# sundy-li/databend

Hardware: AMD Instinct MI355X
Metric: input rows/sec aggregated (filter + hash GROUP BY), % HBM roofline (higher is better)
Workload: dtype int16 key / u64 count; 1 GPU; clickbench_q8_adv_engine_id; rows_per_gpu=100000000, input_copies=4, groups=32, selected_rows=629660, parallelism=single

## Files before the change

databend_amd/csrc/abi.hip:

```cpp
#include "abi_internal.hpp"

static thread_local std::string g_last_error;

int fail(int code, const std::string& msg) {
    g_last_error = msg;
    return code;
}
int abi_fail(int code, const std::string& msg) { return fail(code, msg); }

int err_bits_fail(u64 err, u64 mask) {
    err &= mask;
    if (err & ERR_OVF_LOST) return fail(DBG_ERR_INTERNAL, "overflow list exhausted");
    if (err & ERR_MINMAX_SPIN)
        return fail(DBG_ERR_INTERNAL, "Decimal128 MIN/MAX: a state update gave up after 2^20 contended attempts (the result would be wrong)");
    if (err & ERR_CHAIN_SPIN)
        return fail(DBG_ERR_INTERNAL, "fused finalize: a parked row was not posted in time (GPU hand-off stalled)");
    if (err & ERR_FIXED_INCOMPLETE)
        return fail(DBG_ERR_INVALID, "fixed-capacity exchange incomplete (a partial held more groups than the "
                                     "buffer, or unresolved overflow): use dbg_agg_partition + export_records");
    return DBG_OK;
}

int own_alloc(Owner o, size_t bytes) {
    DevBuf b;
// ... 431 lines not shown
        hipError_t e = hipGetDevice(&h->device);
        if (e != hipSuccess) {
            delete h;
            return fail(DBG_ERR_DEVICE, std::string("hipGetDevice: ") + hipGetErrorString(e));
        }
    }
    auto cleanup = [&](int code) {
        dbg_agg_destroy(h);
        return code;
    };
    if (hipSetDevice(h->device) != hipSuccess) return cleanup(fail(DBG_ERR_DEVICE, "hipSetDevice failed"));
    if (hipStreamCreateWithFlags(&h->own_stream, hipStreamNonBlocking) != hipSuccess) return cleanup(fail(DBG_ERR_DEVICE, "hipStreamCreate failed"));
    h->stream = h->own_stream;
    if ((rc = h->counters.ensure(CNT_WORDS)) != DBG_OK) return cleanup(rc);
    if (hipMemset(h->counters, 0, CNT_WORDS * 8) != hipSuccess) return cleanup(fail(DBG_ERR_DEVICE, "memset"));
    h->spec.err = h->counters + CNT_ERR;
    {
        const char* cx = getenv("DBG_X_PPSPEC_CAP");
        const char* fd = getenv("DBG_X_PPSPEC_DESC");
        h->spec.x_pp_cap = cx ? std::max<u32>(64, (u32)atoi(cx) & ~3u) : ~0u;
        h->spec.x_pp_desc = (fd && fd[0] == '1') ? 1 : 0;
    }
    if ((rc = h->dspec.ensure(1)) != DBG_OK) return cleanup(rc);
    if (hipMemcpy(h->dspec, &h->spec, sizeof(Spec), hipMemcpyHostToDevice) != hipSuccess) return cleanup(fail(DBG_ERR_DEVICE, "spec upload"));
    if ((rc = h->hcounters.ensure(CNT_WORDS + DBG_MAX_KEYS + 8)) != DBG_OK) return cleanup(rc);
    if (hipHostGetDevicePointer((void**)&h->hcounters_dev, h->hcounters.get(), 0) != hipSuccess) h->hcounters_dev = nullptr;
    h->hint_groups = params->capacity_hint;
    u64 hint = params->capacity_hint ? params->capacity_hint : 512;
    h->cap = pow2_at_least(std::max<u64>(hint * 2, 1024));
    h->init_cap = h->cap;
    if ((rc = alloc_table(h, h->cap, h->slots)) != DBG_OK) return cleanup(rc);
    h->scr_blocks = DBG_INSERT_MAX_BLOCKS;
    if ((rc = h->scratch.ensure(scr_words(h->scr_blocks, (u32)h->spec.stride_words))) != DBG_OK) return cleanup(rc);
    if (hipMemset(h->scratch, 0, (size_t)h->scr_blocks * 16) != hipSuccess) return cleanup(fail(DBG_ERR_DEVICE, "memset"));

    BatchDesc* st;
    u32 bid;
    if ((rc = new_batch(h, &st, &bid)) != DBG_OK) return cleanup(rc);
    h->n_batches = 0;
    if (hipStreamSynchronize(h->stream) != hipSuccess) return cleanup(fail(DBG_ERR_DEVICE, "sync"));
    *out = h;
    return DBG_OK;
}

void dbg_agg_destroy(dbg_agg_handle* h) {
    if (!h) return;
    hipSetDevice(h->device);
    if (h->stream) hipStreamSynchronize(h->stream);
    if (h->switch_ev) hipEventDestroy(h->switch_ev);
    if (h->own_stream) hipStreamDestroy(h->own_stream);
    delete h;
}

int dbg_agg_set_stream(dbg_agg_handle* h, void* s) {
    if (!h) return fail(DBG_ERR_INVALID, "null handle");
    HIPCHECK(hipSetDevice(h->device));
    RETURN_IF(flush_deferred(h));
    hipStream_t ns = s ? (hipStream_t)s : h->own_stream;
    if (ns != h->stream) {
        if (!h->switch_ev) HIPCHECK(hipEventCreateWithFlags(&h->switch_ev, hipEventDisableTiming));
        HIPCHECK(hipEventRecord(h->switch_ev, h->stream));
        HIPCHECK(hipStreamWaitEvent(ns, h->switch_ev, 0));
        h->stream = ns;
    }
    return DBG_OK;
}

// ... 132 lines not shown
```

databend_amd/csrc/abi_finalize.hip:

```cpp
#include "abi_exp.hpp"

static void note_observed(dbg_agg_handle* h) {
    const u64 rows = h->table_rows > h->remerged ? h->table_rows - h->remerged : 0;
    if (h->pp || !rows) return;
    h->obs_rows = rows;
    h->obs_groups = h->n_groups;
}

static void publish_groups(const dbg_agg_handle* h, uint64_t* n_groups, uint64_t* string_bytes) {
    if (n_groups) *n_groups = h->n_groups;
    if (string_bytes)
        for (int c = 0; c < h->spec.n_keys; ++c) string_bytes[c] = h->string_bytes[c];
}

bool groups_known(dbg_agg_handle* h, u64 groups, const u64* str_tot, const FinState* caps, uint64_t* n_groups,
                  uint64_t* string_bytes) {
    const Spec& S = h->spec;
    h->n_groups = groups;
    note_observed(h);
    h->string_bytes.assign(S.n_keys, 0);
    bool short_buf = caps && groups > caps->max_groups;
    for (int c = 0; c < S.n_keys; ++c) {
        if (S.key_types[c].type != DBG_STRING) continue;
        h->string_bytes[c] = str_tot[c];
// ... 150 lines not shown
        const u64 total = (size_t)a < h->agg_string_bytes.size() ? h->agg_string_bytes[a] : 0;
        if (on_device && (!out_aggs[a].offsets || (total && !out_aggs[a].data)))
            return fail(DBG_ERR_INVALID, "dbg_agg_result: a String aggregate needs offsets and data buffers");
        u64* offs = nullptr;
        u8* data = nullptr;
        if (dest(out_aggs[a].offsets, (n + 1) * 8, (void**)&offs) != DBG_OK || dest(out_aggs[a].data, total, (void**)&data) != DBG_OK)
            return DBG_ERR_OOM;
        {
            prof::Scope ps("str_gather", h->stream);
            launch_str_gather(h->stream, h->dbatches, a, (const u64*)od.agg_data[a], n, offs, data, total);
        }
        to_host(out_aggs[a].offsets, offs, (n + 1) * 8);
        to_host(out_aggs[a].data, data, total);
    }
    for (int a = 0; a < S.n_aggs && !ser; ++a)
        if (h->result_types[a].nullable) RETURN_IF(pack_validity(od.agg_valid[a], out_aggs[a]));
    for (int c = 0; c < S.n_keys; ++c) {
        const dbg_datatype& t = S.key_types[c];
        to_host(out_keys[c].data, od.key_data[c], t.type == DBG_STRING ? h->string_bytes[c] : n * type_width(t.type));
        if (t.type == DBG_STRING) to_host(out_keys[c].offsets, od.key_offsets[c], (n + 1) * 8);
    }
    for (int a = 0; a < S.n_aggs && !ser; ++a)
        if (!is_str_minmax(S.aggs[a])) to_host(out_aggs[a].data, od.agg_data[a], n * type_width(h->result_types[a].type));
    HIPCHECK(hipMemcpyAsync(h->hcounters, h->counters, CNT_WORDS * 8, hipMemcpyDeviceToHost, h->stream));
    hipError_t e = hipStreamSynchronize(h->stream);
    if (e != hipSuccess) return fail(DBG_ERR_DEVICE, std::string("result: ") + hipGetErrorString(e));
    if (h->hcounters[CNT_ERR] & ERR_DEC_OVERFLOW) {
        HIPCHECK(hipMemsetAsync(h->counters + CNT_ERR, 0, 8, h->stream));
        return fail(DBG_ERR_OVERFLOW, "Decimal overflow");
    }
    return DBG_OK;
}

static int fin_launch(dbg_agg_handle* h) {
    FinState& F = h->fin;
    const Spec& S = h->spec;
    RETURN_IF(stage_flush(h));
    u64 nb = finalize_blocks(h->cap);
    RETURN_IF(h->d_pos.ensure(nb + 16, 1024));
    RETURN_IF(h->d_str_pos.ensure((u64)S.n_keys * nb + 8, 1024));
    const bool direct = h->def_part && !h->pp && S.n_keys == 1 && S.n_aggs == 1 && !S.key_types[0].nullable &&
                        !h->result_types[0].nullable && type_width(h->result_types[0].type) == 8 && F.keys[0].data && F.aggs[0].data &&
                        type_width(S.key_types[0].type) == (u32)h->def_part_kw;
    if (direct) {
        h->def_part = false;
        RETURN_IF(h->part_status.ensure(part_direct_status_words(h->cap, h->def_part_sb), 1024));
    }
    TableDesc t = direct ? TableDesc{} : table_desc(h);
    const bool small = h->cap + 1 <= FIN_SMALL_SLOTS;
    const bool fuse = h->def_on && !h->pp && small && h->hcounters_dev && insert_can_fuse(S, h->def_hb, h->cap);
    if (!fuse) RETURN_IF(flush_deferred(h));
    u64* totals = h->d_pos + nb;
    F.direct = direct;
    if (!small && !h->pp && !direct) count_and_scan(h, t, nb);
    OutDesc od;
    memset(&od, 0, sizeof(od));
    od.cap_groups = F.max_groups;
    u8* vb = h->vbytes;
    for (int c = 0; c < S.n_keys; ++c) {
        od.key_data[c] = F.keys[c].data;
        od.key_offsets[c] = S.key_types[c].type == DBG_STRING ? F.keys[c].offsets : nullptr;
        od.cap_str[c] = (S.key_types[c].type == DBG_STRING && F.has_max_str) ? F.max_str[c] : 0;
        F.cap_str[c] = od.cap_str[c];
        if (S.key_types[c].nullable) {
            od.key_valid[c] = vb;
            od.key_bits[c] = F.keys[c].validity;
            vb += F.max_groups + 1;
        }
    }
    for (int a = 0; a < S.n_aggs; ++a) {
        od.agg_data[a] = F.aggs[a].data;
        if (h->result_types[a].nullable) {
            od.agg_bits[a] = F.aggs[a].validity;
            if (agg_always_valid(S.aggs[a])) {
                od.all_valid |= 1u << a;
            } else {
                od.agg_valid[a] = vb;
                vb += F.max_groups + 1;
            }
        }
    }
    if (h->pp) {
        F.zero_copy = false;
        F.seq = ++h->fin_seq;
        RETURN_IF(pp_fin_launch(h, od));
        F.active = true;
        return DBG_OK;
    }
    F.zero_copy = small && !direct && h->hcounters_dev != nullptr;
    F.seq = ++h->fin_seq;
    if (direct) {
        prof::Scope ps("part_direct", h->stream);
        TableDesc td{};
        td.slots = h->slots;
        td.cap = h->cap;
        hipError_t e = launch_part_direct(h->stream, td, h->def_part_sb, h->part_sorted, h->part_bounds, h->part_status,
                                          h->def_part_kw, od.key_data[0], (u64*)od.agg_data[0], od.cap_groups, totals);
        if (e != hipSuccess) return fail(DBG_ERR_DEVICE, std::string("partitioned insert (direct stage): ") + hipGetErrorString(e));
        launch_finish_outputs(h->stream, od, totals, S.n_keys, S.n_aggs);
    } else if (fuse) {
        FusedFin ff;
        ff.out = od;
        ff.totals = totals;
        ff.host_mirror = h->hcounters_dev;
        ff.seq = F.seq;
        ff.recycle = h->recycle;
        ff.on = 1;
        ff.table_empty = h->def_clean ? 1 : 0;
        ff.trace = nullptr;
        ff.dense = nullptr;
        ff.dense_n = 0;
        RETURN_IF(exp_fused_fin(h, F, ff));
        h->def_on = false;
        prof::Scope ps("agg_insert", h->stream);
        note_insert(h, launch_insert(h->stream, h->dspec, S, h->dbatches, h->def_bid, h->def_rows, false, t, true, &h->def_hb, &ff));
    } else if (small) {
        prof::Scope ps("finalize_small", h->stream);
        launch_finalize_small(h->stream, h->dspec, h->dbatches, t, od, totals, F.zero_copy ? h->hcounters_dev : nullptr,
                              h->recycle && F.zero_copy, F.seq);
    } else {
        prof::Scope ps("write_results", h->stream);
        launch_write_results(h->stream, h->dspec, S, h->dbatches, t, h->d_pos, h->d_str_pos, od);
        launch_finish_outputs(h->stream, od, totals, S.n_keys, S.n_aggs);
    }
    if (!F.zero_copy) {
        HIPCHECK(hipMemcpyAsync(h->hcounters, h->counters, CNT_WORDS * 8, hipMemcpyDeviceToHost, h->stream));
        HIPCHECK(hipMemcpyAsync(h->hcounters + CNT_WORDS, totals, 8 * (S.n_keys + 1), hipMemcpyDeviceToHost, h->stream));
    }
    F.active = true;
    return DBG_OK;
}

static int fin_complete(dbg_agg_handle* h, bool* retry, uint64_t* n_groups, uint64_t* string_bytes) {
    FinState& F = h->fin;
    *retry = false;
    F.active = false;
    if (h->pp) return pp_fin_complete(h, n_groups, string_bytes);
    bool recycled = false;
    const bool direct_done = F.direct;
    if (!F.zero_copy) {
        HIPCHECK(hipStreamSynchronize(h->stream));
    } else {
        volatile u64* hseq = h->hcounters + CNT_WORDS + 2 + DBG_MAX_KEYS;
        volatile u64* hcomp = h->hcounters + MIRROR_COMPACT;
// ... 180 lines not shown
```

databend_amd/csrc/abi_internal.hpp:

```cpp
#pragma once
#include <hip/hip_runtime.h>

#include <algorithm>
#include <cstdio>
#include <cstring>
#include <map>
#include <mutex>
#include <string>
#include <vector>
#include <chrono>

#include "agg.hpp"
#include "dev_buf.hpp"
#include "host_stage.hpp"
#include "legacy.hpp"
#include "serde.hpp"

#include "filter.hpp"
#include "sort.hpp"
#include "prof.hpp"

int fail(int code, const std::string& msg);

#define HIPCHECK(expr)                                                                         \
// ... 62 lines not shown
    u32 n_cached = 0;
    std::vector<std::pair<u64, BatchDesc>> desc_cache;
    std::vector<BatchDesc*> pinned_descs;
    std::vector<PinnedBuf<BatchDesc>> pinned_chunks;
    std::vector<DevBuf> owned;
    DevBuf xrecv[2];
    bool xrecv_busy = false;
    struct XChunk {
        std::vector<u64> pc;
        const void* recv[2] = {nullptr, nullptr};
    };
    std::vector<XChunk> xchunks;
    u32 xfirst[2] = {0, 0};

    bool finalized = false;
    u64 n_groups = 0;
    std::vector<u64> string_bytes;
    std::vector<u64> agg_string_bytes;
    Buf<u64> d_pos;
    Buf<u64> d_str_pos;
    u32 part_n = 0;
    int part_scheme = 0;
    int part_keys = 0;
    u64 part_nb = 0;
    Buf<u64> d_part_pos, d_part_str_pos, d_part_str_base;
    Buf<u64> d_lpart;
    std::vector<u64> part_counts, part_strings;
    Buf<u8> vbytes;
    FinState fin;
    hipEvent_t switch_ev = nullptr;
    int recycle = 0;
    bool clean = false;
    bool init_pending = false;
    u64 fin_seq = 0;
    bool uploads_pending = false;
    Buf<u64> part_sorted, part_bounds;
    Buf<u8> part_temp;
    bool def_part = false;
    u32 def_part_sb = 0;
    int def_part_kw = 0;
    Buf<u64> part_status;
    u64 insert_paths[INS_N_PATHS] = {};
    u64 table_rows = 0;
    u64 remerged = 0;
    int strategy = DBG_STRATEGY_AUTO;
    u64 hint_groups = 0;
    u64 obs_rows = 0, obs_groups = 0;

    bool pp = false;
    double pp_ratio = 1.0;
    double est_groups = 0;
    bool pp_probed = false;
    struct Seg {
        u64 base, n;
        std::vector<u64> off;
    };
    struct Kind {
        Buf<u8> l1;
        u64 l1_n = 0;
        Buf<u16> dig;
        u64 dig_n = 0;
        std::vector<Seg> segs;
        Buf<u8> a, b;
        Buf<u64> part;
        u8* fin = nullptr;
        u8* alt = nullptr;
    } ppk[2];
// ... 106 lines not shown
```

databend_amd/csrc/agg.hip:

```cpp
#include <cstdlib>
#include <cstring>
#include <limits>
#include <type_traits>

#include "legacy.hpp"
#include "agg.hpp"
#include <hip/hip_ext.h>
#include "agg_dev.hpp"

#define BLOCK 256
#define SLOTS_PER_THREAD 8
#define SLOTS_PER_BLOCK (BLOCK * SLOTS_PER_THREAD)
#define LDS_BUDGET_BYTES (32 * 1024)
#define LDS_PROBE_CAP 64
#define FLUSH_ROUND 16



__device__ __forceinline__ u64 pack_key(const Spec& S, const DCol* keys, u64 i) {
    u64 k = 0;
    for (int c = 0; c < S.n_keys; ++c) {
        const DCol& col = keys[c];
        bool v = dcol_valid(col, i);
        if (col.nullable) k |= (u64)(v ? 1 : 0) << (8 * S.voff[c]);
// ... 2101 lines not shown
        const u64 cnt = ld_sc1(gmeta + gg);
        const u64 e = ld_sc1(r);
        const u64 c1 = CO ? ld_sc1(r + 1) : 0;
        if (k >= cnt) continue;
        u64 slot;
        if (view_find(lds, t, e, vclaims, slot)) {
            merge_parked<AS_LDS, CO>(S, batches, lds + slot * sw, r, c1);
        } else {
            push_ovf_rec<true>(S, t, e, r);
            bad = 1;
        }
    }
    if (vclaims) atomicAdd(&vcl, vclaims);
    __syncthreads();
    const bool known = ff.table_empty && ovf_seen == 0 && !bad;
    if (threadIdx.x == 0 && vcl && !(CO && known)) {
        atomicAdd((unsigned long long*)(t.counters + CNT_CLAIMS), (unsigned long long)vcl);
        asm volatile("s_waitcnt vmcnt(0)" ::: "memory");
    }
    __syncthreads();
    if (kPhaseTrace && ff.trace && threadIdx.x == 0) ff.trace[5] = __builtin_amdgcn_s_memrealtime();
    if constexpr (CO) finalize_count_only<T>(t, lds, ff, known, vcl);
    else finalize_small_body<FUSED_FIN_SLOTS / FIN_NT, false>(S, batches, t, lds, ff.out, ff.totals, ff.host_mirror, ff.recycle, ff.seq,
                                                       ff.trace, true);
    if (kPhaseTrace && ff.trace && threadIdx.x == 0) ff.trace[6] = __builtin_amdgcn_s_memrealtime();
}

#ifndef CHAIN_TAGGED
#define CHAIN_TAGGED 1
#endif
constexpr bool kChainTagged = CHAIN_TAGGED != 0;
#define TAG1_BITS 24
#define TAG2_BITS 20
__device__ __forceinline__ u64 chain_pack(u64 key, u64 cnt, u64 seq, int level) {
    const int tb = level == 1 ? TAG1_BITS : TAG2_BITS;
    return key | (cnt << 16) | ((seq & ((1ULL << tb) - 1)) << (64 - tb));
}

template <typename T>
__device__ __forceinline__ void fused_chain_tagged(const Spec& S, const BatchDesc* batches, const BatchDesc& B, u64* lds, u32 lds_slots,
                                                   u32 sw, u32* lcount, u32 nt, const TableDesc& t, u32 my_claims, u32 my_ovf,
                                                   const FusedFin& ff) {
    constexpr int OWN = 4;
    __shared__ u32 role, bad, vcl, wg_ovf;
    __shared__ u64 hbm_claims, ovf_seen;
    const u32 lmask = lds_slots - 1;
    const u32 llimit = lds_slots - lds_slots / 4;
    u64* counts = t.scratch;
    u64* tickets = t.scratch + t.scr_blocks;
    u64* gmeta = tickets + t.scr_blocks / 2;
    u64* rows = t.scratch + 2 * (u64)t.scr_blocks;
    u64* grows = rows + (u64)t.scr_blocks * SCR_ENTRIES * sw;
    const u32 n_groups = (gridDim.x + SCR_GROUP - 1) / SCR_GROUP;
    const u32 g = blockIdx.x / SCR_GROUP;
    const u32 gsize = min((u32)SCR_GROUP, gridDim.x - g * SCR_GROUP);
    const u64 seq = ff.seq & ((1ULL << 44) - 1);
    if (threadIdx.x == 0) wg_ovf = 0;
    __syncthreads();
    auto flush_if_large = [&]() -> bool {
        if (lcount[0] <= SCR_ENTRIES) return false;
        flush_lds_direct<true, false, false, false>(S, batches, B, lds, lds_slots, sw, nt, t, my_claims);
        my_ovf += threadIdx.x == 0 ? 1u : 0u;
        return true;
    };
    auto claims_and_ticket = [&](u64* ticket, u64 carried_claims, u64 carried_ovf) -> u64 {
        if (my_claims) atomicAdd(&lcount[1], my_claims);
        if (my_ovf) atomicAdd(&wg_ovf, my_ovf);
        my_claims = my_ovf = 0;
        asm volatile("s_waitcnt vmcnt(0)" ::: "memory");
        __syncthreads();
        u64 tk = 0;
        if (threadIdx.x == 0) {
            if (lcount[1]) {
                atomicAdd((unsigned long long*)(t.counters + CNT_CLAIMS), (unsigned long long)lcount[1]);
                asm volatile("s_waitcnt vmcnt(0)" ::: "memory");
            }
            const u64 add = 1 + ((carried_claims + lcount[1]) << 16) + ((carried_ovf + wg_ovf) << 40);
            tk = atomicAdd((unsigned long long*)ticket, (unsigned long long)add) + add;
        }
        return tk;
    };
    auto park_tagged = [&](u64* dst, u64* meta, int level) {
        if (threadIdx.x == 0) lcount[2] = 0;
        __syncthreads();
        for (u32 s = threadIdx.x; s < lds_slots; s += nt) {
            const u64* p = lds + (u64)s * sw;
            if (p[0] == SLOT_EMPTY) continue;
            const u32 k = atomicAdd(&lcount[2], 1u);
            st_sc1(dst + k, chain_pack(p[0], p[1], seq, level));
        }
        asm volatile("s_waitcnt vmcnt(0)" ::: "memory");
        __syncthreads();
        if (threadIdx.x == 0) st_sc1(meta, (seq << 20) | lcount[2]);
    };
    auto push_kc = [&](u64 key, u64 c) {
        const u64 k = atomicAdd((unsigned long long*)(t.counters + CNT_OVF_RECS), 1ULL);
        if (k >= t.ovf_recs_cap) {
            atomicOr((unsigned long long*)(t.counters + CNT_ERR), (unsigned long long)ERR_OVF_LOST);
            return;
        }
        u64* r = t.ovf_recs + k * t.stride_words;
        r[0] = key;
        r[1] = c;
    };
    auto read_item = [&](const u64* meta, const u64* row, u32 k, int level, u64& key, u64& cnt) -> bool {
        const int tb = level == 1 ? TAG1_BITS : TAG2_BITS;
        const u64 tag = seq & ((1ULL << tb) - 1);
        for (u32 it = 0; it < (1u << 22); ++it) {
            const u64 m = ld_sc1(meta);
            const u64 w = ld_sc1(row + k);
            if ((m >> 20) == seq) {
                if (k >= (m & 0xFFFFF)) return false;
                if ((w >> (64 - tb)) == tag) {
                    key = w & 0xFFFF;
                    cnt = (w << tb) >> (tb + 16);
                    return true;
                }
            }
            __builtin_amdgcn_s_sleep(1);
        }
        atomicOr((unsigned long long*)(t.counters + CNT_ERR), (unsigned long long)ERR_CHAIN_SPIN);
        bad = 1;
        return false;
    };
    bool flushed = flush_if_large();
    {
        const u64 tk = claims_and_ticket(tickets + g, 0, 0);
        if (threadIdx.x == 0) {
            role = (tk & 0xFFFF) == gsize ? 1u : 0u;
            hbm_claims = (tk >> 16) & 0xFFFFFF;
            ovf_seen = tk >> 40;
            wg_ovf = 0;
            bad = 0;
        }
    }
    __syncthreads();
    if (!role) {
        if (flushed) {
            if (threadIdx.x == 0) st_sc1(counts + blockIdx.x, seq << 20);
        } else {
            park_tagged(rows + (u64)blockIdx.x * SCR_ENTRIES * sw, counts + blockIdx.x, 1);
        }
        return;
    }
    if (threadIdx.x == 0) {
        tickets[g] = 0;
        lcount[1] = 0;
        if (flushed) lcount[0] = 0;
    }
    if (flushed) lds_table_init<false>(S, lds, lds_slots, sw, nt);
    __syncthreads();
    for (u32 f = threadIdx.x; f < gsize * SCR_ENTRIES; f += nt) {
        const u64 b = (u64)g * SCR_GROUP + f / SCR_ENTRIES;
        if (b == blockIdx.x) continue;
        u64 key, c;
        if (!read_item(counts + b, rows + b * SCR_ENTRIES * sw, f % SCR_ENTRIES, 1, key, c)) continue;
        const int ls = lds_find<true>(S, batches, B.keys, 0, key, 0, lds, lmask, sw, lcount, llimit);
        if (ls >= 0) {
            at_add<AS_LDS>(asp<AS_LDS>(lds + (u64)ls * sw + 1), c);
            continue;
        }
        bool claimed;
        const u64 gs = g_find<true>(S, batches, B.keys, 0, key, 0, t, t.probe_limit, claimed);
        if (gs == ~0ULL) {
            push_kc(key, c);
            my_ovf++;
            continue;
        }
        my_claims += claimed ? 1 : 0;
        at_add<AS_GLB>(asp<AS_GLB>(t.slots + gs * t.stride_words + 1), c);
    }
    __syncthreads();
    flushed = flush_if_large();
    {
        const u64 tk = claims_and_ticket(t.counters + CNT_FIN_TICKET, hbm_claims, ovf_seen);
        if (threadIdx.x == 0) {
            role = (tk & 0xFFFF) == n_groups ? 2u : 0u;
            hbm_claims = (tk >> 16) & 0xFFFFFF;
            ovf_seen = tk >> 40;
        }
    }
    __syncthreads();
    if (kPhaseTrace && ff.trace && threadIdx.x == 0) atomicMax((unsigned long long*)ff.trace + 3, (unsigned long long)__builtin_amdgcn_s_memrealtime());
    if (role != 2) {
        if (flushed) {
            if (threadIdx.x == 0) st_sc1(gmeta + g, seq << 20);
        } else {
            park_tagged(grows + (u64)g * SCR_ENTRIES * sw, gmeta + g, 2);
        }
        return;
    }
    if (threadIdx.x == 0) {
        atomicExch((unsigned long long*)(t.counters + CNT_FIN_TICKET), 0ULL);
        atomicExch((unsigned long long*)(t.counters + CNT_TAIL), 0ULL);
        vcl = 0;
        if (kPhaseTrace && ff.trace) ff.trace[4] = __builtin_amdgcn_s_memrealtime();
    }
    u64 okey[OWN], ocnt[OWN];
#pragma unroll
    for (int j = 0; j < OWN; ++j) {
        const u32 s = threadIdx.x + (u32)j * nt;
        okey[j] = SLOT_EMPTY;
        ocnt[j] = 0;
        if (!flushed && s < lds_slots) {
            okey[j] = lds[(u64)s * sw];
            ocnt[j] = lds[(u64)s * sw + 1];
        }
    }
    __syncthreads();
    const u64 n = (t.cap + 1) * sw;
    const bool hbm_clean = ff.table_empty && hbm_claims == 0;
    if (hbm_clean)
        for (u64 i = threadIdx.x; i < n; i += nt) lds[i] = (i % sw) == 0 ? SLOT_EMPTY : 0ULL;
    else
        for (u64 i = threadIdx.x; i < n; i += nt) lds[i] = ld_sc1(t.slots + i);
    __syncthreads();
    u32 vclaims = 0;
    auto to_view = [&](u64 key, u64 c) {
        u64 slot;
        if (view_find(lds, t, key, vclaims, slot)) {
            at_add<AS_LDS>(asp<AS_LDS>(lds + slot * sw + 1), c);
        } else {
            push_kc(key, c);
            bad = 1;
        }
    };
#pragma unroll
    for (int j = 0; j < OWN; ++j)
        if (okey[j] != SLOT_EMPTY) to_view(okey[j], ocnt[j]);
    for (u32 f = threadIdx.x; f < n_groups * SCR_ENTRIES; f += nt) {
        const u64 gg = f / SCR_ENTRIES;
        if (gg == g) continue;
        u64 key, c;
        if (read_item(gmeta + gg, grows + gg * SCR_ENTRIES * sw, f % SCR_ENTRIES, 2, key, c)) to_view(key, c);
    }
    if (vclaims) atomicAdd(&vcl, vclaims);
    __syncthreads();
    const bool known = ff.table_empty && ovf_seen == 0 && !bad;
    if (threadIdx.x == 0 && vcl && !known) {
        atomicAdd((unsigned long long*)(t.counters + CNT_CLAIMS), (unsigned long long)vcl);
        asm volatile("s_waitcnt vmcnt(0)" ::: "memory");
    }
    __syncthreads();
    if (kPhaseTrace && ff.trace && threadIdx.x == 0) ff.trace[5] = __builtin_amdgcn_s_memrealtime();
    finalize_count_only<T>(t, lds, ff, known, vcl, hbm_clean && !bad);
    if (kPhaseTrace && ff.trace && threadIdx.x == 0) ff.trace[6] = __builtin_amdgcn_s_memrealtime();
}

#ifndef FAST_UNROLL
#define FAST_UNROLL 2
#endif
#ifndef TAIL_ON
#define TAIL_ON 0
#endif
typedef unsigned int v4u __attribute__((ext_vector_type(4)));
typedef const v4u __attribute__((address_space(1)))* gv4p;

template <typename T>
__device__ __forceinline__ bool fast_pred(T v, int op, i64 c) {
    T k = (T)c;
    switch (op) {
        case DBG_CMP_EQ: return v == k;
        case DBG_CMP_NE: return v != k;
        case DBG_CMP_LT: return v < k;
        case DBG_CMP_LE: return v <= k;
        case DBG_CMP_GT: return v > k;
        default: return v >= k;
    }
}

template <typename T>
// ... 299 lines not shown
            handle_group(yc, bases, FAST_UNROLL, actm);
#pragma unroll
            for (int u = 0; u < FAST_UNROLL; ++u) yc[u] = yn[u];
            cur = nxt;
        }
    }
    if (PRED && vqn) {
        __builtin_amdgcn_wave_barrier();
        drain_vec(vqn);
    }
    if (PRED && qn) {
        __builtin_amdgcn_wave_barrier();
        if (lane < (int)qn) process(((vwptr<AS_LDS>)qkey)[lane], ((vwptr<AS_LDS>)qrow)[lane]);
        qn = 0;
    }
    for (u64 i = nvec * V + (u64)blockIdx.x * NT + threadIdx.x; i < rows; i += gstride) {
        T v = gld<T>(col + i);
        if (!PRED || pass(v)) process((u64)(typename std::make_unsigned<T>::type)v, i);
    }
    __syncthreads();
    if (kPhaseTrace && ff.trace && threadIdx.x == 0) {
        const u64 tm = __builtin_amdgcn_s_memrealtime();
        atomicMin((unsigned long long*)ff.trace + 1, (unsigned long long)tm);
        atomicMax((unsigned long long*)ff.trace + 2, (unsigned long long)tm);
    }
    if constexpr (CO && sizeof(T) <= 2) {
        if (ff.on && ff.dense && t.scratch != nullptr && gridDim.x > 1 && gridDim.x < 65536) {
            fused_dense<T>(S, batches, B, lds, lds_slots, sw, lcount, NT, t, my_claims, my_ovf, ff);
            return;
        }
    }
    if (ff.on && t.scratch != nullptr && gridDim.x > 1 && gridDim.x <= t.scr_blocks) {
        if constexpr (CO && sizeof(T) <= 2) {
            if (kChainTagged && lds_slots <= 4 * NT) {
                fused_chain_tagged<T>(S, batches, B, lds, lds_slots, sw, lcount, NT, t, my_claims, my_ovf, ff);
                return;
            }
        }
        fused_chain<T, CO>(S, batches, B, lds, lds_slots, sw, lcount, NT, t, my_claims, my_ovf, ff);
        return;
    }
    block_flush<true, false, false, false>(S, batches, B, lds, lds_slots, sw, lcount, NT, t, my_claims);
    if (kPhaseTrace && ff.trace && threadIdx.x == 0) atomicMax((unsigned long long*)ff.trace + 3, (unsigned long long)__builtin_amdgcn_s_memrealtime());
    if (ff.on) fused_finalize(S, batches, t, lds, ff);
}


bool prof_ext_events(hipEvent_t* a, hipEvent_t* b);

static size_t fast_shmem(size_t table_bytes) { return table_bytes + (size_t)(1024 / 64) * WQW * 8; }
static size_t fast_table_bytes(const Spec& S) { return (size_t)lds_slots_for(S, 16 * 1024) * S.stride_words * 8 + 16; }

template <typename T>
static void launch_fast_t(hipStream_t s, const Spec* dspec, const BatchDesc* batches, u32 bid, u64 rows, const TableDesc& t,
                          u32 lslots, size_t table_bytes, bool pred, int op, i64 c, int count_only, const FusedFin* fused) {
    constexpr u64 V = 16 / sizeof(T);
    typedef __int128 W;
    const W tmin = (W)std::numeric_limits<T>::min(), tmax = (W)std::numeric_limits<T>::max();
    const W C = std::is_signed<T>::value ? (W)c : (W)(u64)c;
    W lo = 1, hi = 0;
    int neg = 0;
    auto all = [&]() { lo = tmin; hi = tmax; };
    switch (op) {
        case DBG_CMP_EQ: if (C >= tmin && C <= tmax) lo = hi = C; break;
        case DBG_CMP_NE: neg = 1; if (C >= tmin && C <= tmax) lo = hi = C; break;
        case DBG_CMP_LT: if (C > tmax) all(); else if (C > tmin) { lo = tmin; hi = C - 1; } break;
        case DBG_CMP_LE: if (C >= tmax) all(); else if (C >= tmin) { lo = tmin; hi = C; } break;
        case DBG_CMP_GT: if (C < tmin) all(); else if (C < tmax) { lo = C + 1; hi = tmax; } break;
        default: if (C <= tmin) all(); else if (C <= tmax) { lo = C; hi = tmax; } break;
    }
    if (lo > hi) { lo = 1; hi = 0; }
    const int nt = 1024;
    static_assert(FIN_NT == 1024, "the fused finalize runs on the insert's workgroup");
    static const u64 x_grid = X_ENV("DBG_X_FAST_GRID") ? (u64)atoll(X_ENV("DBG_X_FAST_GRID")) : 0;
    const u64 max_blocks = (x_grid && fused && fused->dense) ? x_grid : 256;
    size_t shmem = fast_shmem(table_bytes);
    FusedFin ff;
    if (fused) ff = *fused;
    else memset(&ff, 0, sizeof(ff));
    u64 quantum = V * (u64)nt * FAST_UNROLL;
    u64 blocks = (rows + quantum - 1) / quantum;
    if (blocks > max_blocks) blocks = max_blocks;
    if (blocks > DBG_INSERT_MAX_BLOCKS) blocks = DBG_INSERT_MAX_BLOCKS;
    if (blocks < 1) blocks = 1;
    hipEvent_t ev0 = nullptr, ev1 = nullptr;
    const bool ext = prof_ext_events(&ev0, &ev1);
#define FAST_LAUNCH(P, N, F)                                                                                                     \
    do {                                                                                                                         \
        if (ext)                                                                                                                 \
            hipExtLaunchKernelGGL((agg_insert_fast_kernel<T, P, N, F>), dim3((u32)blocks), dim3(N), shmem, s, ev0, ev1, 0, dspec, \
                                  batches, bid, rows, t, lslots, (T)lo, (T)hi, neg, ff);                                        \
        else                                                                                                                     \
            hipLaunchKernelGGL((agg_insert_fast_kernel<T, P, N, F>), dim3((u32)blocks), dim3(N), shmem, s, dspec, batches, bid, \
                               rows, t, lslots, (T)lo, (T)hi, neg, ff);                                                          \
    } while (0)
    if (count_only) {
        if (pred) FAST_LAUNCH(true, 1024, true); else FAST_LAUNCH(false, 1024, true);
    } else {
        if (pred) FAST_LAUNCH(true, 1024, false); else FAST_LAUNCH(false, 1024, false);
    }
#undef FAST_LAUNCH
}

static bool fast_eligible(const Spec& S, const BatchDesc& hb, bool records) {
    if (records || !S.inline_keys || S.n_keys != 1 || S.key_types[0].nullable) return false;
    for (int a = 0; a < S.n_aggs; ++a)
        if ((S.aggs[a].kind == DBG_AGG_MIN || S.aggs[a].kind == DBG_AGG_MAX) && S.aggs[a].mmk == MMK_STR) return false;
    for (int a = 0; a < S.n_aggs; ++a)
        if (S.aggs[a].arg_type == DBG_DECIMAL256) return false;
    const DCol& k = hb.keys[0];
    int ty = k.type;
    bool intlike = (ty >= DBG_INT8 && ty <= DBG_UINT64) || ty == DBG_DATE || ty == DBG_TIMESTAMP;
    if (!intlike || k.layout != LAYOUT_ARROW || ((uintptr_t)k.data & 15)) return false;
    if (hb.n_nodes == 0) return true;
    if (hb.n_nodes != 1) return false;
    const DNode& n = hb.nodes[0];
    const DCol& f = hb.fcols[n.col];
// ... 453 lines not shown
```

databend_amd/csrc/agg.hpp:

```cpp
#pragma once
#include "device.hpp"

#define SLOT_EMPTY 0xFFFFFFFFFFFFFFFFULL
#define KC_KEY_WORDS 4

struct Spec {
    int32_t n_keys;
    int32_t inline_keys;
    int32_t inline_width;
    int32_t n_aggs;
    int32_t n_words;
    int32_t stride_words;
    int32_t tstride;
    int32_t kc_word;
    int32_t flags_word;
    int32_t has_strings;
    uint8_t voff[DBG_MAX_KEYS];
    uint8_t koff[DBG_MAX_KEYS];
    dbg_datatype key_types[DBG_MAX_KEYS];
    uint32_t rec_width;
    uint32_t rec_key_off[DBG_MAX_KEYS];
    uint32_t rec_val_off[DBG_MAX_KEYS];
    uint32_t rec_state_off;
    DAgg aggs[DBG_MAX_AGGS];
// ... 21 lines not shown
    int32_t is_records;
    uint32_t rec_width;
    const u8* rec_base;
    u64 seg_records;
    DCol keys[DBG_MAX_KEYS];
    DCol args[DBG_MAX_AGGS];
    DCol fcols[DBG_MAX_FCOLS];
    DNode nodes[DBG_MAX_NODES];
};

struct TableDesc {
    u64* slots;
    u64 cap;
    u32 stride_words;
    u32 probe_limit;
    u64* counters;
    u64* ovf_rows;
    u64 ovf_rows_cap;
    u64* ovf_recs;
    u64 ovf_recs_cap;
    u64* scratch;
    u32 scr_blocks;
};
#define SCR_ENTRIES 64
#ifndef SCR_GROUP
#define SCR_GROUP 16
#endif
#ifndef FLUSH_GROUP
#define FLUSH_GROUP 4
#endif
inline size_t scr_words(u32 blocks, u32 stride_words) {
    return (size_t)blocks * (2 + (size_t)SCR_ENTRIES * stride_words) + (size_t)(blocks / SCR_GROUP) * SCR_ENTRIES * stride_words;
}
#define DBG_INSERT_MAX_BLOCKS 2048

enum { CNT_CLAIMS = 0, CNT_OVF_ROWS = 1, CNT_OVF_RECS = 2, CNT_ERR = 3, CNT_FIX_FAIL = 4, CNT_FIX_TICKET = 5, CNT_FIN_TICKET = 6,
       CNT_TAIL = 7, CNT_WORDS = 8 };
enum { ERR_DEC_OVERFLOW = 1, ERR_OVF_LOST = 2, ERR_FIXED_INCOMPLETE = 4, ERR_MINMAX_SPIN = 8, ERR_CHAIN_SPIN = 16 };

__host__ __device__ __forceinline__ u64 slot_mix(u64 x) { return hash_prim(x ^ 0x9E3779B97F4A7C15ULL); }
constexpr u64 mul_inverse_u64(u64 c) {
    u64 x = c;
    for (int i = 0; i < 6; ++i) x *= 2 - c * x;
    return x;
}
__host__ __device__ __forceinline__ u64 slot_unmix(u64 y) {
    constexpr u64 CI = mul_inverse_u64(0xd6e8feb86659fd93ULL);
    y ^= y >> 32;
    y *= CI;
    y ^= y >> 32;
    y *= CI;
    y ^= y >> 32;
    return y ^ 0x9E3779B97F4A7C15ULL;
}
static_assert(0xd6e8feb86659fd93ULL * mul_inverse_u64(0xd6e8feb86659fd93ULL) == 1, "inverse");

#define AS_GLB 1
#define AS_LDS 3
template <int AS> using wptr = __attribute__((address_space(AS))) u64*;
template <int AS> using sptr = __attribute__((address_space(AS))) long long*;
template <int AS> using dptr = __attribute__((address_space(AS))) double*;
template <int AS> using vwptr = volatile __attribute__((address_space(AS))) u64*;
template <int AS> __device__ __forceinline__ wptr<AS> asp(u64* p) { return (wptr<AS>)p; }
template <int AS> __device__ __forceinline__ wptr<AS> asp(const u64* p) { return (wptr<AS>)(u64*)p; }
#define AT_SCOPE(AS) ((AS) == AS_LDS ? __HIP_MEMORY_SCOPE_WORKGROUP : __HIP_MEMORY_SCOPE_AGENT)
template <int AS> __device__ __forceinline__ u64 at_add(wptr<AS> p, u64 v) {
// ... 121 lines not shown
    u64* key_offsets[DBG_MAX_KEYS];
    u8* key_valid[DBG_MAX_KEYS];
    void* agg_data[DBG_MAX_AGGS];
    u8* agg_valid[DBG_MAX_AGGS];
    u64 cap_groups;
    u64 cap_str[DBG_MAX_KEYS];
    u8* key_bits[DBG_MAX_KEYS];
    u8* agg_bits[DBG_MAX_AGGS];
    int32_t ser;
    u32 ser_stride[DBG_MAX_AGGS];
    u32 all_valid;
};
__host__ __device__ __forceinline__ u8 all_valid_byte(u64 n, u64 k) {
    const u64 i0 = k * 8;
    return i0 + 8 <= n ? (u8)0xFF : (i0 < n ? (u8)((1u << (n - i0)) - 1) : (u8)0);
}
void launch_fill_valid(hipStream_t s, u64 n, u8* bits);
#define FIN_SMALL_SLOTS 16384
void launch_finalize_small(hipStream_t s, const Spec* dspec, const BatchDesc* batches, const TableDesc& t, const OutDesc& out,
                           u64* totals, u64* host_mirror ,
                           int recycle, u64 seq);
void launch_finish_outputs(hipStream_t s, const OutDesc& out, const u64* totals, int n_keys, int n_aggs);
void launch_ser_compact(hipStream_t s, const u8* lens, const u8* src, u32 stride, u64 n, u64* offs, u8* dst, u64* total);
#define FUSED_FIN_SLOTS 2048
#define MIRROR_COMPACT (CNT_WORDS + 3 + DBG_MAX_KEYS)
struct FusedFin {
    OutDesc out;
    u64* totals;
    u64* host_mirror;
    u64 seq;
    int recycle;
    int on;
    int table_empty;
    u64* trace;
    u64* dense;
    u32 dense_n;
};
bool insert_can_fuse(const Spec& S, const BatchDesc& hb, u64 cap);
void launch_write_results(hipStream_t s, const Spec* dspec, const Spec& hspec, const BatchDesc* batches, const TableDesc& t,
                          const u64* pos , const u64* str_pos, const OutDesc& out);
void launch_pack_bits(hipStream_t s, const u8* bytes, u64 n, u8* bits);
void launch_str_agg_bytes(hipStream_t s, const Spec* dspec, const BatchDesc* batches, const TableDesc& t, u64* totals);
void launch_str_gather(hipStream_t s, const BatchDesc* batches, int a, const u64* refs, u64 n, u64* offs, u8* data, u64 cap_bytes);
void launch_export_fixed(hipStream_t s, const Spec* dspec, const BatchDesc* batches, const TableDesc& t, u8* buf, u64 cap_records,
                         int recycle);
void launch_export(hipStream_t s, const Spec* dspec, const Spec& hspec, const BatchDesc* batches, const TableDesc& t,
                   u32 n_parts, int scheme, const u32* lpart, const u64* pos, const u64* str_pos, u8* rec_out, u8* str_out,
                   const u64* part_str_base);

struct PPChunk {
    u64 start;
    u64 n;
    u32 bid;
    u32 group;
};
#define PP_L1_BITS 8
#define PP_CHUNK 262144
#define PP_NT 512
#define PP_SCRATCH_BYTES (32 * 1024)
__host__ __device__ __forceinline__ u32 pp_direct_t(u32 rw) {
    const u32 t = PP_SCRATCH_BYTES / rw;
    return t >= PP_NT ? PP_NT : (t & ~63u);
}
void launch_pp_sample(hipStream_t s, const Spec* dspec, const BatchDesc* batches, u32 bid, u64 rows, u64 n_sample,
                      u64* set, u64 set_cap, u64* out);
void launch_pp_count(hipStream_t s, const Spec* dspec, const BatchDesc* batches, int src, int kind, const u8* src_recs,
// ... 69 lines not shown
```

Baseline: 2434 billion rows/s.

## Restructure fused chain-tagged finalize hand-off with prefetch, one-item-per-thread merge and LDS fast path

Reworks the fused two-level chain-tagged finalize. Each workgroup now parks its entries before taking the ticket, and each thread prefetches one peer item in parallel instead of looping over all items. The final workgroup writes results straight from LDS when the table is clean. Tag-wrap safety is also added: the sequence counter skips zero low bits, the host clears scratch at each tag period, and the path is gated on block count and count-width limits. The aim is to cut serialized barriers and spin latency at the tail of the aggregation, at the cost of more complex correctness conditions.

```diff
diff --git a/databend_amd/csrc/abi.hip b/databend_amd/csrc/abi.hip
--- a/databend_amd/csrc/abi.hip
+++ b/databend_amd/csrc/abi.hip
@@ -487,7 +487,8 @@
     if ((rc = alloc_table(h, h->cap, h->slots)) != DBG_OK) return cleanup(rc);
     h->scr_blocks = DBG_INSERT_MAX_BLOCKS;
     if ((rc = h->scratch.ensure(scr_words(h->scr_blocks, (u32)h->spec.stride_words))) != DBG_OK) return cleanup(rc);
-    if (hipMemset(h->scratch, 0, (size_t)h->scr_blocks * 16) != hipSuccess) return cleanup(fail(DBG_ERR_DEVICE, "memset"));
+    if (hipMemset(h->scratch, 0, scr_words(h->scr_blocks, (u32)h->spec.stride_words) * 8) != hipSuccess)
+        return cleanup(fail(DBG_ERR_DEVICE, "memset"));
 
     BatchDesc* st;
     u32 bid;
diff --git a/databend_amd/csrc/abi_finalize.hip b/databend_amd/csrc/abi_finalize.hip
--- a/databend_amd/csrc/abi_finalize.hip
+++ b/databend_amd/csrc/abi_finalize.hip
@@ -206,6 +206,11 @@
     return DBG_OK;
 }
 
+static u64 next_fin_seq(dbg_agg_handle* h) {
+    if ((++h->fin_seq & (FIN_SEQ_TAG_PERIOD - 1)) == 0) ++h->fin_seq;
+    return h->fin_seq;
+}
+
 static int fin_launch(dbg_agg_handle* h) {
     FinState& F = h->fin;
     const Spec& S = h->spec;
@@ -256,13 +261,13 @@
     }
     if (h->pp) {
         F.zero_copy = false;
-        F.seq = ++h->fin_seq;
+        F.seq = next_fin_seq(h);
         RETURN_IF(pp_fin_launch(h, od));
         F.active = true;
         return DBG_OK;
     }
     F.zero_copy = small && !direct && h->hcounters_dev != nullptr;
-    F.seq = ++h->fin_seq;
+    F.seq = next_fin_seq(h);
     if (direct) {
         prof::Scope ps("part_direct", h->stream);
         TableDesc td{};
@@ -281,9 +286,14 @@
         ff.recycle = h->recycle;
         ff.on = 1;
         ff.table_empty = h->def_clean ? 1 : 0;
+        ff.chain_tagged = 0;
         ff.trace = nullptr;
         ff.dense = nullptr;
         ff.dense_n = 0;
+        if ((F.seq / FIN_SEQ_TAG_PERIOD) != h->scr_period) {
+            HIPCHECK(hipMemsetAsync(h->scratch, 0, scr_words(h->scr_blocks, (u32)S.stride_words) * 8, h->stream));
+            h->scr_period = F.seq / FIN_SEQ_TAG_PERIOD;
+        }
         RETURN_IF(exp_fused_fin(h, F, ff));
         h->def_on = false;
         prof::Scope ps("agg_insert", h->stream);
diff --git a/databend_amd/csrc/abi_internal.hpp b/databend_amd/csrc/abi_internal.hpp
--- a/databend_amd/csrc/abi_internal.hpp
+++ b/databend_amd/csrc/abi_internal.hpp
@@ -118,7 +118,8 @@
     int recycle = 0;
     bool clean = false;
     bool init_pending = false;
-    u64 fin_seq = 0;
+    u64 fin_seq = (1ULL << 24) - 32;
+    u64 scr_period = ((1ULL << 24) - 32) / FIN_SEQ_TAG_PERIOD;
     bool uploads_pending = false;
     Buf<u64> part_sorted, part_bounds;
     Buf<u8> part_temp;
diff --git a/databend_amd/csrc/agg.hip b/databend_amd/csrc/agg.hip
--- a/databend_amd/csrc/agg.hip
+++ b/databend_amd/csrc/agg.hip
@@ -2157,9 +2157,39 @@
 constexpr bool kChainTagged = CHAIN_TAGGED != 0;
 #define TAG1_BITS 24
 #define TAG2_BITS 20
+#define CNT1_BITS (64 - 16 - TAG1_BITS)
+#define CNT2_BITS (64 - 16 - TAG2_BITS)
+static_assert(FIN_SEQ_TAG_PERIOD == (1ULL << TAG2_BITS), "the host clears the scratch when the narrower tag wraps");
+static_assert(TAG2_BITS <= TAG1_BITS, "the host keeps the low TAG2_BITS of the sequence number non-zero: both tags then are");
+static_assert(((u64)SCR_GROUP << CNT1_BITS) <= (1ULL << CNT2_BITS), "a group's count fits a level-2 entry");
+static_assert(SCR_GROUP * SCR_ENTRIES <= FIN_NT, "one parked item per thread at level 1");
+#define CHAIN_TAGGED_MAX_BLOCKS (SCR_GROUP * (FIN_NT / SCR_ENTRIES))
 __device__ __forceinline__ u64 chain_pack(u64 key, u64 cnt, u64 seq, int level) {
     const int tb = level == 1 ? TAG1_BITS : TAG2_BITS;
     return key | (cnt << 16) | ((seq & ((1ULL << tb) - 1)) << (64 - tb));
+}
+
+template <typename T, int OWN>
+__device__ __forceinline__ void finalize_count_lds(const TableDesc& t, const u64* lds, u32 lds_slots, u32 sw, u32 nt, u32* next,
+                                                   u32 total, const FusedFin& ff) {
+    const OutDesc& out = ff.out;
+#pragma unroll
+    for (int j = 0; j < OWN; ++j) {
+        const u32 s = threadIdx.x + (u32)j * nt;
+        if (s >= lds_slots) continue;
+        const u64 e = lds[(u64)s * sw];
+        if (e == SLOT_EMPTY) continue;
+        const u32 p = atomicAdd(next, 1u);
+        if (p >= out.cap_groups) continue;
+        ((T*)out.key_data[0])[p] = (T)e;
+        ((u64*)out.agg_data[0])[p] = lds[(u64)s * sw + 1];
+    }
+    if (threadIdx.x < CNT_WORDS) t.counters[threadIdx.x] = 0;
+    if (threadIdx.x == 0) {
+        ff.totals[0] = total;
+        __hip_atomic_store(ff.host_mirror + MIRROR_COMPACT, (ff.seq << 25) | (1ULL << 24) | total, __ATOMIC_RELAXED,
+                           __HIP_MEMORY_SCOPE_SYSTEM);
+    }
 }
 
 template <typename T>
@@ -2167,7 +2197,7 @@
                                                    u32 sw, u32* lcount, u32 nt, const TableDesc& t, u32 my_claims, u32 my_ovf,
                                                    const FusedFin& ff) {
     constexpr int OWN = 4;
-    __shared__ u32 role, bad, vcl, wg_ovf;
+    __shared__ u32 role, bad, vcl;
     __shared__ u64 hbm_claims, ovf_seen;
     const u32 lmask = lds_slots - 1;
     const u32 llimit = lds_slots - lds_slots / 4;
@@ -2180,43 +2210,55 @@
     const u32 g = blockIdx.x / SCR_GROUP;
     const u32 gsize = min((u32)SCR_GROUP, gridDim.x - g * SCR_GROUP);
     const u64 seq = ff.seq & ((1ULL << 44) - 1);
-    if (threadIdx.x == 0) wg_ovf = 0;
-    __syncthreads();
-    auto flush_if_large = [&]() -> bool {
-        if (lcount[0] <= SCR_ENTRIES) return false;
-        flush_lds_direct<true, false, false, false>(S, batches, B, lds, lds_slots, sw, nt, t, my_claims);
-        my_ovf += threadIdx.x == 0 ? 1u : 0u;
-        return true;
+    auto lds_barrier = [] { asm volatile("s_waitcnt lgkmcnt(0)\n\ts_barrier" ::: "memory"); };
+    auto post_claims = [&]() {
+        if (my_claims) atomicAdd(&lcount[1], my_claims);
+        if (my_ovf) atomicOr(&lcount[3], 1u);
+        my_claims = my_ovf = 0;
     };
-    auto claims_and_ticket = [&](u64* ticket, u64 carried_claims, u64 carried_ovf) -> u64 {
-        if (my_claims) atomicAdd(&lcount[1], my_claims);
-        if (my_ovf) atomicAdd(&wg_ovf, my_ovf);
-        my_claims = my_ovf = 0;
+    auto settle_hbm = [&]() -> bool {
+        const bool large = lcount[0] > SCR_ENTRIES;
+        if (large) {
+            flush_lds_direct<true, false, false, false>(S, batches, B, lds, lds_slots, sw, nt, t, my_claims);
+            if (threadIdx.x == 0) atomicOr(&lcount[3], 1u);
+        }
+        post_claims();
         asm volatile("s_waitcnt vmcnt(0)" ::: "memory");
         __syncthreads();
+        if (threadIdx.x == 0 && lcount[1]) {
+            atomicAdd((unsigned long long*)(t.counters + CNT_CLAIMS), (unsigned long long)lcount[1]);
+            asm volatile("s_waitcnt vmcnt(0)" ::: "memory");
+        }
+        return large;
+    };
+    auto hand_off = [&](u64* ticket, u64 carried_claims, u64 carried_ovf, bool flushed, u64* dst, u64* meta, int level,
+                        bool others, const u64* o_meta, const u64* o_ent, u64& m, u64& w) -> u64 {
+        m = w = 0;
+        if (others) {
+            m = ld_sc1(o_meta);
+            w = ld_sc1(o_ent);
+        }
+        u64 old, add = 0;
+        if (threadIdx.x == 0) {
+            add = 1 + ((carried_claims + lcount[1]) << 16) + ((u64)((carried_ovf || lcount[3]) ? 1 : 0) << 40);
+            asm volatile("global_atomic_add_x2 %0, %1, %2, off sc0" : "=&v"(old) : "v"(ticket), "v"(add) : "memory");
+        }
+        if (!flushed)
+            for (u32 s = threadIdx.x; s < lds_slots; s += nt) {
+                const u64* p = lds + (u64)s * sw;
+                if (p[0] == SLOT_EMPTY) continue;
+                const u32 k = atomicAdd(&lcount[2], 1u);
+                st_sc1(dst + k, chain_pack(p[0], p[1], seq, level));
+            }
+        lds_barrier();
         u64 tk = 0;
         if (threadIdx.x == 0) {
-            if (lcount[1]) {
-                atomicAdd((unsigned long long*)(t.counters + CNT_CLAIMS), (unsigned long long)lcount[1]);
-                asm volatile("s_waitcnt vmcnt(0)" ::: "memory");
-            }
-            const u64 add = 1 + ((carried_claims + lcount[1]) << 16) + ((carried_ovf + wg_ovf) << 40);
-            tk = atomicAdd((unsigned long long*)ticket, (unsigned long long)add) + add;
+            st_sc1(meta, (seq << 20) | lcount[2]);
+            lcount[1] = lcount[2] = lcount[3] = 0;
+            asm volatile("s_waitcnt vmcnt(0)" : "+v"(old) : : "memory");
+            tk = old + add;
         }
         return tk;
-    };
-    auto park_tagged = [&](u64* dst, u64* meta, int level) {
-        if (threadIdx.x == 0) lcount[2] = 0;
-        __syncthreads();
-        for (u32 s = threadIdx.x; s < lds_slots; s += nt) {
-            const u64* p = lds + (u64)s * sw;
-            if (p[0] == SLOT_EMPTY) continue;
-            const u32 k = atomicAdd(&lcount[2], 1u);
-            st_sc1(dst + k, chain_pack(p[0], p[1], seq, level));
-        }
-        asm volatile("s_waitcnt vmcnt(0)" ::: "memory");
-        __syncthreads();
-        if (threadIdx.x == 0) st_sc1(meta, (seq << 20) | lcount[2]);
     };
     auto push_kc = [&](u64 key, u64 c) {
         const u64 k = atomicAdd((unsigned long long*)(t.counters + CNT_OVF_RECS), 1ULL);
@@ -2228,12 +2270,10 @@
         r[0] = key;
         r[1] = c;
     };
-    auto read_item = [&](const u64* meta, const u64* row, u32 k, int level, u64& key, u64& cnt) -> bool {
+    auto take_item = [&](const u64* meta, const u64* ent, u32 k, int level, u64 m, u64 w, u64& key, u64& cnt) -> bool {
         const int tb = level == 1 ? TAG1_BITS : TAG2_BITS;
         const u64 tag = seq & ((1ULL << tb) - 1);
         for (u32 it = 0; it < (1u << 22); ++it) {
-            const u64 m = ld_sc1(meta);
-            const u64 w = ld_sc1(row + k);
             if ((m >> 20) == seq) {
                 if (k >= (m & 0xFFFFF)) return false;
                 if ((w >> (64 - tb)) == tag) {
@@ -2241,85 +2281,114 @@
                     cnt = (w << tb) >> (tb + 16);
                     return true;
                 }
-            }
+            } else {
+                m = ld_sc1(meta);
+            }
+            w = ld_sc1(ent);
             __builtin_amdgcn_s_sleep(1);
         }
         atomicOr((unsigned long long*)(t.counters + CNT_ERR), (unsigned long long)ERR_CHAIN_SPIN);
         bad = 1;
+        atomicOr(&lcount[3], 1u);
         return false;
     };
-    bool flushed = flush_if_large();
-    {
-        const u64 tk = claims_and_ticket(tickets + g, 0, 0);
-        if (threadIdx.x == 0) {
-            role = (tk & 0xFFFF) == gsize ? 1u : 0u;
-            hbm_claims = (tk >> 16) & 0xFFFFFF;
-            ovf_seen = tk >> 40;
-            wg_ovf = 0;
-            bad = 0;
-        }
-    }
-    __syncthreads();
-    if (!role) {
-        if (flushed) {
-            if (threadIdx.x == 0) st_sc1(counts + blockIdx.x, seq << 20);
-        } else {
-            park_tagged(rows + (u64)blockIdx.x * SCR_ENTRIES * sw, counts + blockIdx.x, 1);
-        }
-        return;
-    }
-    if (threadIdx.x == 0) {
-        tickets[g] = 0;
-        lcount[1] = 0;
-        if (flushed) lcount[0] = 0;
-    }
-    if (flushed) lds_table_init<false>(S, lds, lds_slots, sw, nt);
-    __syncthreads();
-    for (u32 f = threadIdx.x; f < gsize * SCR_ENTRIES; f += nt) {
-        const u64 b = (u64)g * SCR_GROUP + f / SCR_ENTRIES;
-        if (b == blockIdx.x) continue;
-        u64 key, c;
-        if (!read_item(counts + b, rows + b * SCR_ENTRIES * sw, f % SCR_ENTRIES, 1, key, c)) continue;
+    auto merge_item = [&](u64 key, u64 c) {
         const int ls = lds_find<true>(S, batches, B.keys, 0, key, 0, lds, lmask, sw, lcount, llimit);
         if (ls >= 0) {
             at_add<AS_LDS>(asp<AS_LDS>(lds + (u64)ls * sw + 1), c);
-            continue;
+            return;
         }
         bool claimed;
         const u64 gs = g_find<true>(S, batches, B.keys, 0, key, 0, t, t.probe_limit, claimed);
         if (gs == ~0ULL) {
             push_kc(key, c);
             my_ovf++;
-            continue;
+            return;
         }
         my_claims += claimed ? 1 : 0;
         at_add<AS_GLB>(asp<AS_GLB>(t.slots + gs * t.stride_words + 1), c);
-    }
-    __syncthreads();
-    flushed = flush_if_large();
+    };
+    auto empty_own = [&]() {
+        lds_table_init<false>(S, lds, lds_slots, sw, nt);
+        if (threadIdx.x == 0) lcount[0] = 0;
+        __syncthreads();
+    };
+    const u32 item_row = threadIdx.x / SCR_ENTRIES, item_k = threadIdx.x % SCR_ENTRIES;
+    post_claims();
+    asm volatile("s_waitcnt vmcnt(0)" ::: "memory");
+    lds_barrier();
+    bool flushed = false;
+    if (lcount[1] | lcount[3] | (lcount[0] > SCR_ENTRIES ? 1u : 0u)) flushed = settle_hbm();
+    const u64 b1 = (u64)g * SCR_GROUP + item_row;
+    const bool has1 = item_row < gsize && b1 != blockIdx.x;
+    const u64* meta1 = counts + b1;
+    const u64* ent1 = rows + b1 * SCR_ENTRIES * sw + item_k;
+    u64 m1, w1;
     {
-        const u64 tk = claims_and_ticket(t.counters + CNT_FIN_TICKET, hbm_claims, ovf_seen);
+        const u64 tk = hand_off(tickets + g, 0, 0, flushed, rows + (u64)blockIdx.x * SCR_ENTRIES * sw, counts + blockIdx.x, 1, has1,
+                                meta1, ent1, m1, w1);
+        if (threadIdx.x == 0) {
+            role = (tk & 0xFFFF) == gsize ? 1u : 0u;
+            hbm_claims = (tk >> 16) & 0xFFFFFF;
+            ovf_seen = tk >> 40;
+            bad = 0;
+            vcl = 0;
+        }
+    }
+    lds_barrier();
+    if (!role) return;
+    if (threadIdx.x == 0) tickets[g] = 0;
+    if (flushed) empty_own();
+    {
+        u64 key, c;
+        if (has1 && take_item(meta1, ent1, item_k, 1, m1, w1, key, c)) merge_item(key, c);
+    }
+    post_claims();
+    asm volatile("s_waitcnt vmcnt(0)" ::: "memory");
+    lds_barrier();
+    flushed = false;
+    if (lcount[1] | lcount[3] | (lcount[0] > SCR_ENTRIES ? 1u : 0u)) flushed = settle_hbm();
+    const bool has2 = item_row < n_groups && item_row != g;
+    const u64* meta2 = gmeta + item_row;
+    const u64* ent2 = grows + (u64)item_row * SCR_ENTRIES * sw + item_k;
+    u64 m2, w2;
+    {
+        const u64 tk = hand_off(t.counters + CNT_FIN_TICKET, hbm_claims, ovf_seen, flushed, grows + (u64)g * SCR_ENTRIES * sw, gmeta + g,
+                                2, has2, meta2, ent2, m2, w2);
         if (threadIdx.x == 0) {
             role = (tk & 0xFFFF) == n_groups ? 2u : 0u;
             hbm_claims = (tk >> 16) & 0xFFFFFF;
             ovf_seen = tk >> 40;
         }
     }
-    __syncthreads();
+    lds_barrier();
     if (kPhaseTrace && ff.trace && threadIdx.x == 0) atomicMax((unsigned long long*)ff.trace + 3, (unsigned long long)__builtin_amdgcn_s_memrealtime());
-    if (role != 2) {
-        if (flushed) {
-            if (threadIdx.x == 0) st_sc1(gmeta + g, seq << 20);
-        } else {
-            park_tagged(grows + (u64)g * SCR_ENTRIES * sw, gmeta + g, 2);
-        }
-        return;
-    }
+    if (role != 2) return;
     if (threadIdx.x == 0) {
         atomicExch((unsigned long long*)(t.counters + CNT_FIN_TICKET), 0ULL);
         atomicExch((unsigned long long*)(t.counters + CNT_TAIL), 0ULL);
-        vcl = 0;
         if (kPhaseTrace && ff.trace) ff.trace[4] = __builtin_amdgcn_s_memrealtime();
+    }
+    if (flushed) empty_own();
+    {
+        u64 key, c;
+        if (has2 && take_item(meta2, ent2, item_k, 2, m2, w2, key, c)) merge_item(key, c);
+    }
+    post_claims();
+    asm volatile("s_waitcnt vmcnt(0)" ::: "memory");
+    __syncthreads();
+    const u32 own_groups = lcount[0], spill_claims = lcount[1], spill_ovf = lcount[3];
+    const bool ovf_any = ovf_seen != 0 || spill_ovf != 0;
+    if (ff.table_empty && hbm_claims == 0 && spill_claims == 0 && !ovf_any && !bad && ff.recycle && ff.host_mirror &&
+        own_groups <= ff.out.cap_groups) {
+        if (kPhaseTrace && ff.trace && threadIdx.x == 0) ff.trace[5] = __builtin_amdgcn_s_memrealtime();
+        finalize_count_lds<T, OWN>(t, lds, lds_slots, sw, nt, &lcount[2], own_groups, ff);
+        if (kPhaseTrace && ff.trace && threadIdx.x == 0) ff.trace[6] = __builtin_amdgcn_s_memrealtime();
+        return;
+    }
+    if (threadIdx.x == 0 && spill_claims) {
+        atomicAdd((unsigned long long*)(t.counters + CNT_CLAIMS), (unsigned long long)spill_claims);
+        asm volatile("s_waitcnt vmcnt(0)" ::: "memory");
     }
     u64 okey[OWN], ocnt[OWN];
 #pragma unroll
@@ -2327,14 +2396,14 @@
         const u32 s = threadIdx.x + (u32)j * nt;
         okey[j] = SLOT_EMPTY;
         ocnt[j] = 0;
-        if (!flushed && s < lds_slots) {
+        if (s < lds_slots) {
             okey[j] = lds[(u64)s * sw];
             ocnt[j] = lds[(u64)s * sw + 1];
         }
     }
     __syncthreads();
     const u64 n = (t.cap + 1) * sw;
-    const bool hbm_clean = ff.table_empty && hbm_claims == 0;
+    const bool hbm_clean = ff.table_empty && hbm_claims == 0 && spill_claims == 0;
     if (hbm_clean)
         for (u64 i = threadIdx.x; i < n; i += nt) lds[i] = (i % sw) == 0 ? SLOT_EMPTY : 0ULL;
     else
@@ -2353,15 +2422,9 @@
 #pragma unroll
     for (int j = 0; j < OWN; ++j)
         if (okey[j] != SLOT_EMPTY) to_view(okey[j], ocnt[j]);
-    for (u32 f = threadIdx.x; f < n_groups * SCR_ENTRIES; f += nt) {
-        const u64 gg = f / SCR_ENTRIES;
-        if (gg == g) continue;
-        u64 key, c;
-        if (read_item(gmeta + gg, grows + gg * SCR_ENTRIES * sw, f % SCR_ENTRIES, 2, key, c)) to_view(key, c);
-    }
     if (vclaims) atomicAdd(&vcl, vclaims);
     __syncthreads();
-    const bool known = ff.table_empty && ovf_seen == 0 && !bad;
+    const bool known = ff.table_empty && !ovf_any && !bad;
     if (threadIdx.x == 0 && vcl && !known) {
         atomicAdd((unsigned long long*)(t.counters + CNT_CLAIMS), (unsigned long long)vcl);
         asm volatile("s_waitcnt vmcnt(0)" ::: "memory");
@@ -2727,7 +2790,7 @@
     }
     if (ff.on && t.scratch != nullptr && gridDim.x > 1 && gridDim.x <= t.scr_blocks) {
         if constexpr (CO && sizeof(T) <= 2) {
-            if (kChainTagged && lds_slots <= 4 * NT) {
+            if (kChainTagged && ff.chain_tagged && lds_slots <= 4 * NT) {
                 fused_chain_tagged<T>(S, batches, B, lds, lds_slots, sw, lcount, NT, t, my_claims, my_ovf, ff);
                 return;
             }
@@ -2778,6 +2841,8 @@
     if (blocks > max_blocks) blocks = max_blocks;
     if (blocks > DBG_INSERT_MAX_BLOCKS) blocks = DBG_INSERT_MAX_BLOCKS;
     if (blocks < 1) blocks = 1;
+    static_assert(FAST_UNROLL >= 1 && V * 1024 * FAST_UNROLL < (1ULL << CNT1_BITS), "one grid round of a workgroup fits a level-1 count");
+    ff.chain_tagged = blocks <= CHAIN_TAGGED_MAX_BLOCKS && rows / blocks + V * (u64)nt + V < (1ULL << CNT1_BITS);
     hipEvent_t ev0 = nullptr, ev1 = nullptr;
     const bool ext = prof_ext_events(&ev0, &ev1);
 #define FAST_LAUNCH(P, N, F)                                                                                                     \
diff --git a/databend_amd/csrc/agg.hpp b/databend_amd/csrc/agg.hpp
--- a/databend_amd/csrc/agg.hpp
+++ b/databend_amd/csrc/agg.hpp
@@ -77,6 +77,7 @@
 inline size_t scr_words(u32 blocks, u32 stride_words) {
     return (size_t)blocks * (2 + (size_t)SCR_ENTRIES * stride_words) + (size_t)(blocks / SCR_GROUP) * SCR_ENTRIES * stride_words;
 }
+#define FIN_SEQ_TAG_PERIOD (1ULL << 20)
 #define DBG_INSERT_MAX_BLOCKS 2048
 
 enum { CNT_CLAIMS = 0, CNT_OVF_ROWS = 1, CNT_OVF_RECS = 2, CNT_ERR = 3, CNT_FIX_FAIL = 4, CNT_FIX_TICKET = 5, CNT_FIN_TICKET = 6,
@@ -264,6 +265,7 @@
     int recycle;
     int on;
     int table_empty;
+    int chain_tagged;
     u64* trace;
     u64* dense;
     u32 dense_n;
```

Measured after the change: 2543 billion rows/s (median of 6 runs). 1.04x the previous value.
